# ArchieGertsman/spark-sched-sim

Measured on AMD Instinct MI355X. Metric: env-steps/sec at 4096 batched envs (TPC-H, 10 exec), higher is better.
Workload: dtype int64+f64

## Files before the change

### spark_sched_sim_amd/csrc/sss_sim.h

```cpp
#pragma once
#ifdef SSS_WIDE
#ifdef SSS_TIMELINE
#define SSS_KNAME(name) name##_wide_tl
#else
#define SSS_KNAME(name) name##_wide
#endif
#else
#ifdef SSS_TIMELINE
#define SSS_KNAME(name) name##_tl
#else
#define SSS_KNAME(name) name
#endif
#endif
#include "../../include/sss.h"
#include "sss_layout.h"
#include <wave_rt.h>


struct alignas(16) SssScratch {
  uint8_t pool8[8];
  uint8_t pool8b[8];
  uint64_t rng_buf[64];
  int32_t rng_pos, pad0_[3];
  uint8_t setA[SSS_SET_TABLE];
// ... 120 lines not shown
    if (H.err == 0) H.err = (code), H.err_line = (uint64_t)SSS_SRC_ID * 100000u + __LINE__; \
  } while (0)
#endif
#ifdef SSS_CHECK_TRACE
#define CHECK(cond)                                                                     \
  do {                                                                                  \
    if (!(cond)) {                                                                      \
      if (H.err == 0) fprintf(stderr, "[CHECK] line %d: %s\n", __LINE__, #cond);         \
      FAIL(SSS_ERR_INVARIANT);                                                          \
    }                                                                                   \
  } while (0)
#else
#define CHECK(cond)                          \
  do {                                       \
    if (!(cond)) FAIL(SSS_ERR_INVARIANT);     \
  } while (0)
#endif

#if defined(__HIP_DEVICE_COMPILE__) || defined(__clang__)
#define SSS_UNROLL4 _Pragma("unroll 4")
#define SSS_UNROLL8 _Pragma("unroll 8")
#else
#define SSS_UNROLL4
#define SSS_UNROLL8
#endif

#ifdef SSS_BATCH_STATS
extern "C" { extern long long sss_batch_stats[128]; }
#define STAT(i, v) ((void)(wave_lane() == 0 ? (sss_batch_stats[i] += (v)) : 0))
#else
#define STAT(i, v) ((void)0)
#endif

#include "sss_prof.h"
#if defined(SSS_CHECK_TRACE) && defined(SSS_UTRACE)
#define UTRACE(tag) do { if (wave_lane() < 2 && getenv("SSS_UTRACE")) fprintf(stderr, "[u] lane %d %s\n", wave_lane(), tag); } while (0)
#else
#define UTRACE(tag) ((void)0)
#endif

#define LENW_LEN 0x3FFFFFFF
#define SLOT_NONE 255
SSS_DEV uint16_t* lds_active() { return (uint16_t*)(g_pool + g_c.P.off_active); }
SSS_DEV uint8_t* lds_slot_of() { return g_pool + g_c.P.off_slot_of; }
SSS_DEV uint16_t* lds_keys() { return (uint16_t*)(g_pool + g_c.P.off_keys); }
SSS_DEV uint16_t* lds_jobset() { return (uint16_t*)(g_pool + g_c.P.off_jobset); }
SSS_DEV SssJob* lds_cjobs() { return (SssJob*)(g_pool + g_c.P.off_cjobs); }
SSS_DEV SssStage* lds_cstages() { return (SssStage*)(g_pool + g_c.P.off_cstages); }
SSS_DEV float* lds_cdur() { return (float*)(g_pool + g_c.P.off_cdur); }
SSS_DEV SssExDesc* lds_exdesc() { return (SssExDesc*)(g_pool + g_c.P.off_exdesc); }
SSS_DEV uint16_t* lds_old_active() { return (uint16_t*)(g_pool + g_c.P.off_old_active); }
SSS_DEV uint16_t* lds_slot_job() { return (uint16_t*)(g_pool + g_c.P.off_slot_job); }
SSS_DEV uint8_t* lds_slot_ref() { return g_pool + g_c.P.off_slot_ref; }

SSS_DEV SssJob* jobp(int j) {
  int s = lds_slot_of()[j];
  return s != SLOT_NONE ? lds_cjobs() + s : g_c.jobs + j;
}
SSS_DEV SssStage* stgp(int j, int st) {
  int s = lds_slot_of()[j];
  return s != SLOT_NONE ? lds_cstages() + s * g_c.SP + st : g_c.stages + j * g_c.SP + st;
}
SSS_DEV float* durp(int j, int st) {
  int s = lds_slot_of()[j];
  return s != SLOT_NONE ? lds_cdur() + s * g_c.SP + st : g_c.durations + j * g_c.SP + st;
}
// ... 443 lines not shown
```

### spark_sched_sim_amd/csrc/sss_sim_env.h

```cpp
#undef SSS_SRC_ID
#define SSS_SRC_ID 11
SSS_DEV void env_begin(const uint8_t* base) {
  PROF3(23);
  int lane = wave_lane();
  {
    const SssHot* g = (const SssHot*)base;
    if (lane < (int)(sizeof(SssHdr) / 16)) ((uint4*)&g_hot.h)[lane] = ((const uint4*)&g->h)[lane];
    for (int x = lane; x < SSS_MAX_EXEC; x += 64) {
      SssEvSlot ev;
      ev.t = __builtin_inf(), ev.seq = 0, ev.info = EV_NONE;
      uint32_t loc = POOL_NONE, csrc = 0, cdst = 0, cseq = 0;
      int16_t job = -1, cn = 0;
      int8_t ts = -1;
      uint8_t exe = 0;
      if (x < g_c.E)
        ev = g->ev[x], loc = g->ex_loc[x], job = g->ex_job[x], ts = g->ex_task_stage[x], exe = g->ex_executing[x], csrc = g->c_src[x],
        cdst = g->c_dst[x], cseq = g->c_seq[x], cn = g->c_n[x];
      g_hot.ev[x] = ev, g_hot.ex_loc[x] = loc, g_hot.ex_job[x] = job, g_hot.ex_task_stage[x] = ts, g_hot.ex_executing[x] = exe;
      g_hot.c_src[x] = csrc, g_hot.c_dst[x] = cdst, g_hot.c_seq[x] = cseq, g_hot.c_n[x] = cn;
    }
  }
  for (int i = lane; i < g_c.J_cap; i += 64) lds_slot_of()[i] = SLOT_NONE;
  for (int x = lane; x < g_c.E; x += 64) lds_exdesc()[x].gs = -1;
  lds_slot_ref()[lane] = 0;
// ... 27 lines not shown
      }
    }
    int nK = 0;
    for (int h = 0; h < SSS_EPL; h++) {
      key[h] = first[h] ? ((cnt[h] << 8) | (uint32_t)(64 * SSS_EPL - 1 - (lane + 64 * h))) : 0u;
      nK += popc64(wave_ballot(first[h]));
    }
    for (int h2 = 0; h2 < SSS_EPL; h2++)
      for (uint64_t fm = wave_ballot(first[h2]); fm; fm &= fm - 1) {
        const uint32_t kq = wave_readlane_u32(key[h2], ctz64_nz(fm));
        for (int h = 0; h < SSS_EPL; h++) rank[h] += kq > key[h] ? 1u : 0u;
      }
    const int n_used = nK < g_c.P.n_slots ? nK : g_c.P.n_slots;
    for (int h = 0; h < SSS_EPL; h++)
      if (first[h] && (int)rank[h] < g_c.P.n_slots) {
        lds_slot_of()[j[h]] = (uint8_t)rank[h];
        lds_slot_job()[rank[h]] = (uint16_t)j[h];
        lds_slot_ref()[rank[h]] = (uint8_t)cnt[h];
      }
    wave_sync();
    for (int h = 0; h < SSS_EPL; h++)
      if (has[h]) g_hot.ev[lane + 64 * h].info = info_with_slot(info[h], (uint32_t)lds_slot_of()[j[h]]);
    if (lane == 0) {
      uint64_t all = g_c.P.n_slots >= 64 ? ~0ull : (bit64(g_c.P.n_slots) - 1);
      uint64_t used = n_used >= 64 ? ~0ull : (bit64(n_used) - 1);
      g_sc.free_slots = all & ~used;
      g_sc.pending_free = -1, g_sc.pinned_job = -1, g_sc.idle_valid = 0, g_sc.fi_detach = 0;
      g_sc.events_this_step = 0;
      g_sc.active_version = 0, g_sc.old_version = 0, g_sc.jobset_valid = 0, g_sc.active_dirty = 0;
      g_sc.rng_pos = 64;
    }
  }
  wave_sync();
  uint64_t occ = ~g_sc.free_slots & (g_c.P.n_slots >= 64 ? ~0ull : (bit64(g_c.P.n_slots) - 1));
  int nK = popc64(occ);
  int per = 8 + g_c.SP + g_c.SP / 2;
  for (int i0 = lane; i0 < nK * per; i0 += 64 * 8) {
    uint64_t v[8];
    SSS_UNROLL8 for (int u = 0; u < 8; u++) {
      const int i = i0 + 64 * u;
      v[u] = 0;
      if (i < nK * per) {
        const int k = i / per, w = i - k * per;
        const int j = lds_slot_job()[k];
        v[u] = w < 8 ? ((const uint64_t*)(g_c.jobs + j))[w]
             : (w < 8 + g_c.SP ? ((const uint64_t*)(g_c.stages + j * g_c.SP))[w - 8] : ((const uint64_t*)(g_c.durations + j * g_c.SP))[w - 8 - g_c.SP]);
      }
    }
    SSS_UNROLL8 for (int u = 0; u < 8; u++) {
      const int i = i0 + 64 * u;
      if (i < nK * per) {
        const int k = i / per, w = i - k * per;
        if (w < 8)
          ((uint64_t*)(lds_cjobs() + k))[w] = v[u];
        else if (w < 8 + g_c.SP)
          ((uint64_t*)(lds_cstages() + k * g_c.SP))[w - 8] = v[u];
        else
          ((uint64_t*)(lds_cdur() + k * g_c.SP))[w - 8 - g_c.SP] = v[u];
      }
    }
  }
  wave_sync();
}

SSS_DEV void env_begin_readonly(const uint8_t* base) {
  int lane = wave_lane();
  const SssHot* g = (const SssHot*)base;
  if (lane < (int)(sizeof(SssHdr) / 16)) ((uint4*)&g_hot.h)[lane] = ((const uint4*)&g->h)[lane];
  for (int i = lane; i < g_c.J_cap; i += 64) lds_slot_of()[i] = SLOT_NONE;
  wave_sync();
  int A = g_hot.h.n_active;
  for (int i = lane; i < A; i += 64) lds_active()[i] = g_c.active_g[i];
  wave_sync();
}

SSS_DEV void env_end(uint8_t* base) {
  PROF3(24);
  int lane = wave_lane();
  wave_sync();
  if (lane == 0) rng_canonicalize();
  int A = g_hot.h.n_active;
  int per = 8 + g_c.SP + g_c.SP / 2;
  uint64_t occ = ~g_sc.free_slots & (g_c.P.n_slots >= 64 ? ~0ull : (bit64(g_c.P.n_slots) - 1));
  for (int i = lane; i < g_c.P.n_slots * per; i += 64) {
    int k = i / per, w = i - k * per;
    if (!(occ & bit64(k))) continue;
    int j = lds_slot_job()[k];
    if (w < 8)
      ((uint64_t*)(g_c.jobs + j))[w] = ((const uint64_t*)(lds_cjobs() + k))[w];
    else if (w < 8 + g_c.SP)
      ((uint64_t*)(g_c.stages + j * g_c.SP))[w - 8] = ((const uint64_t*)(lds_cstages() + k * g_c.SP))[w - 8];
    else
      ((uint64_t*)(g_c.durations + j * g_c.SP))[w - 8 - g_c.SP] = ((const uint64_t*)(lds_cdur() + k * g_c.SP))[w - 8 - g_c.SP];
  }
  if (g_sc.active_dirty)
// ... 15 lines not shown
  }
}


SSS_DEV void select_stage_wave(int stage_idx) {
  PROF3(34);
  const int lane = wave_lane();
  const int A = g_hot.h.n_active;
  int run = 0, fj = -1, fs = -1;
  for (int a0 = 0; a0 < A && stage_idx >= 0; a0 += 64) {
    const int a = a0 + lane;
    uint64_t m = 0;
    int jj = -1;
    if (a < A) jj = lds_active()[a], m = jobp(jj)->sched_mask;
    const uint32_t n = (uint32_t)popc64(m);
    const int lo = run + (int)wave_scan_excl_u32(n);
    run += (int)wave_sum_u32(n);
    const bool mine = stage_idx >= lo && stage_idx < lo + (int)n;
    const uint64_t hit = wave_ballot(mine);
    if (hit) {
      if (mine) {
        for (int i = 0; i < stage_idx - lo; i++) m &= m - 1;
        g_sc.sel_job = jj, g_sc.sel_stage = ctz64(m);
      }
      fj = 0;
      break;
    }
  }
  if (fj < 0 && lane == 0) g_sc.sel_job = -1, g_sc.sel_stage = -1;
  (void)fs;
  wave_sync();
}

SSS_DEV bool take_action(int stage_idx, int num_exec) {
  PROF3(17);
  if (stage_idx < -1 || stage_idx >= H.obs_n_nodes || num_exec < 1 || num_exec > g_c.E) {
    H.err = SSS_ERR_ACTION_SPACE;
    return false;
  }
  if (stage_idx == -1) {
    commit_remaining_executors();
    return true;
  }
  if (stage_idx >= H.obs_n_sched) {
    H.err = SSS_ERR_STAGE_IDX;
    return false;
  }
  if (num_exec > trk_num_committable()) {
    H.err = SSS_ERR_TOO_MANY;
    return false;
  }
  const int j = g_sc.sel_job, s = g_sc.sel_stage;
  CHECK(j >= 0);
  if (j < 0) return false;
  SssStage st = (*stgp(j, s));
  int demand = (int)st.remaining - ((int)st.moving_to + (int)st.commit_to);
  int n = num_exec < demand ? num_exec : demand;
  CHECK(n > 0);
  trk_add_commitment(n, key_stage_pool(j, s));
  SssJob& job = (*jobp(j));
  job.selected_mask |= bit64(s);
  int old_n = popc64(job.sched_mask);
  uint64_t m = 0;
  if (job_passes_filter(j, trk_source_job_id())) m = ready_mask_of_job(job, false);
  job.sched_mask = m;
  H.n_sched += popc64(m) - old_n;
  return true;
}

SSS_DEV void jobtime_build_set() {
  PROF3(18);
  SetImg<uint16_t> all;
  all.tab = lds_jobset();
  for (int i = 0; i < 8; i++) all.tab[i] = 0;
  all.mask = 7, all.fill = 0, all.used = 0, all.finger = 0, all.cap = 0xFFFFFFFFu, all.big = nullptr, all.small = nullptr, all.wide = false;
  for (int k = 0; k < g_sc.n_old_active; k++) set_add(all, (uint32_t)lds_old_active()[k], lds_keys());
  for (int k = 0; k < H.n_active; k++) set_add(all, (uint32_t)lds_active()[k], lds_keys());
  g_sc.jobset_mask = (int32_t)all.mask;
}

SSS_DEV void jobtime_build_set_wave() {
  const int lane = wave_lane();
  uint16_t* tab = lds_jobset();
  const int cap = g_c.P.jobset_slots;
  const int n_old = g_sc.n_old_active, n_act = g_hot.h.n_active;
  for (int i = lane * 8; i < cap; i += 64 * 8) *(uint4*)(tab + i) = mk_u4(0u, 0u, 0u, 0u);
  wave_sync();
  uint32_t not_max = 0xFFFFFFFFu;
  for (int k = lane; k < n_old + n_act; k += 64) {
    const uint32_t id = k < n_old ? lds_old_active()[k] : lds_active()[k - n_old];
    tab[id] = (uint16_t)(id + 2);
    not_max = ~id < not_max ? ~id : not_max;
  }
  wave_sync();
  uint32_t cnt = 0;
  for (int i = lane * 8; i < cap; i += 64 * 8) {
    const uint4 q = *(const uint4*)(tab + i);
    const uint32_t w[4] = {q.x, q.y, q.z, q.w};
    for (int b = 0; b < 4; b++) cnt += ((w[b] & 0xFFFFu) != 0 ? 1u : 0u) + ((w[b] >> 16) != 0 ? 1u : 0u);
// ... 136 lines not shown
          handled = fast_run<FUSED>(f);
        } else if (tasks_left) {
          handled = fast_run<FUSED>(f);
        } else {
#ifndef SSS_NO_BATCH
          if (64 - g_sc.rng_pos < rng_need) {
            rng_refill();
          }
#endif
          handled = tf ? batch_released_events(f, ex) : batch_arrival_events(f, ex);
#ifndef SSS_NO_LEAN
          if (handled == 0) handled = tf ? lean_released(f, ex, t_win, info_win) : lean_arrival(f, ex, t_win, info_win);
#endif
          if (handled == 0 && tf) preflush_completing_job(f, info_win, t_win);
        }
        if (handled > 0) continue;
      }
      if (lane == 0) status = handle_popped(f, ex, t_win, info_win, t_slow);
      status = (int)wave_lane0_u32((uint32_t)status);
    } while (status == 0);
    if (lane == 0) {
      g_sc.f_done = status == 1, g_sc.f_scan = status == 2;
      H.prof[0] += t_slow;
    }
    wave_sync();
    if (g_sc.f_done) {
      if (lane == 0) {
        for (int a = 0; a < H.n_active; a++) (*jobp(lds_active()[a])).sched_mask = 0;
        H.n_sched = 0;
      }
      wave_sync();
      return false;
    }
    int n = find_schedulable_all();
    if (n > 0) {
      if (lane == 0) H.n_sched = n;
      wave_sync();
      return false;
    }
    publish_idle_mask();
    if (lane == 0) {
      move_idle_executors_all(POOL_NONE);
      H.curr_source = POOL_NONE;
      g_sc.idle_valid = 0;
    }
    wave_sync();
  }
}

SSS_DEV void do_reset(const SssLayout& L, uint64_t seed, double time_limit) {
  PROF3(27);
  int lane = wave_lane();
  SssHot& hot = g_hot;
  for (int i = lane; i < g_c.J_cap; i += 64) lds_slot_of()[i] = SLOT_NONE;
  lds_slot_ref()[lane] = 0;
  wave_sync();
  if (lane == 0) {
    g_sc.free_slots = g_c.P.n_slots >= 64 ? ~0ull : (bit64(g_c.P.n_slots) - 1);
    g_sc.pending_free = -1, g_sc.pinned_job = -1, g_sc.idle_valid = 0, g_sc.fi_detach = 0;
    uint64_t n_steps = H.n_steps, n_events = H.n_events, model_bytes = H.model_bytes;
    int dur_head = H.dur_head, dur_n = H.dur_n, episodes = H.episodes, last_ep_steps = H.last_ep_steps;
    double last_ep_return = H.last_ep_return, last_ep_wall = H.last_ep_wall;
    uint64_t prof[5];
    for (int i = 0; i < 5; i++) prof[i] = H.prof[i];
    uint64_t n_fast_keep = H.n_fast, n_batched_keep = H.n_batched, n_rounds_keep = H.n_rounds, pad0_keep = H.err_line;
    SssHdr z = {};
    H = z;
// ... 121 lines not shown
    g_sc.wall_old = H.wall_old, g_sc.n_old_active = H.n_old_active;
    g_sc.old_version = g_sc.active_version, g_sc.jobset_valid = 0;
    H.mid_step = 0;
  }
  wave_sync();
}
SSS_DEV void step_yield() {
  const int lane = wave_lane();
  for (int a = lane; a < g_sc.n_old_active; a += 64) g_c.active_g[g_c.J_cap + a] = lds_old_active()[a];
  if (lane == 0) H.mid_step = 1, H.step_events = g_sc.events_this_step, H.wall_old = g_sc.wall_old, H.n_old_active = g_sc.n_old_active;
  wave_sync();
}

template <bool FUSED = false>
SSS_DEV double do_step(int stage_idx, int num_exec, int budget = 0, bool* yielded = nullptr) {
  PROF3(28);
  int lane = wave_lane();
  uint64_t t0 = wave_clock();
  const bool go_on = wave_ballot(g_hot.h.mid_step != 0) != 0;
  uint64_t t1 = t0;
  if (go_on) {
    step_continue();
  } else {
  publish_idle_mask();
  select_stage_wave(stage_idx);
  if (lane == 0) {
    g_sc.f_round_continues = 1, g_sc.f_fulfil = 0;
    g_sc.events_this_step = 0, g_sc.events_at_launch = 0;
    H.last_reward = 0.0;
    if (H.need_reset || H.terminated) {
      H.err = SSS_ERR_NEED_RESET;
    } else {
      H.err = 0;
      bool ok = take_action(stage_idx, num_exec);
      if (ok && !H.err) {
        H.n_steps++;
        H.ep_steps++;
        if (!(trk_num_committable() > 0 && H.n_sched > 0)) {
          commit_remaining_executors();
          g_sc.f_fulfil = 1;
        }
      }
    }
    if (!g_sc.f_fulfil) g_sc.idle_valid = 0;
  }
  wave_sync();
  if (g_sc.f_fulfil) {
    fulfil_order_commitments();
    if (lane == 0) {
      fulfil_build_list();
      g_sc.idle_valid = 0;
    }
    wave_sync();
    fulfil_run();
    if (lane == 0) {
      H.curr_source = POOL_NONE;
      g_sc.wall_old = H.wall_time;
      g_sc.n_old_active = H.n_active;
      g_sc.old_version = g_sc.active_version;
      g_sc.f_round_continues = 0;
    }
  }
  if (lane == 0 && H.err && H.err != SSS_ERR_ACTION_SPACE && H.err != SSS_ERR_STAGE_IDX && H.err != SSS_ERR_TOO_MANY) H.need_reset = 1;
  wave_sync();
  t1 = wave_clock();
  if (lane == 0) H.prof[1] += t1 - t0;
  if (wave_ballot(g_sc.f_round_continues || g_hot.h.err) != 0) return 0.0;
  for (int a = lane; a < g_hot.h.n_active; a += 64) {
    int j = lds_active()[a];
    (*jobp(j)).selected_mask = 0;
    lds_old_active()[a] = (uint16_t)j;
  }
  wave_sync();
  }
  if (resume_simulation<FUSED>(budget)) {
    step_yield();
    *yielded = true;
    return 0.0;
  }
  return step_reward(t1, wave_clock());
}

SSS_DEV double step_reward(uint64_t t1, uint64_t t2) {
  const int lane = wave_lane();
  if (lane == 0) {
    g_sc.f_need_jobtime = 0;
    if (!H.err && H.wall_time - g_sc.wall_old != 0.0) {
// ... 31 lines not shown
```

### spark_sched_sim_amd/csrc/sss_sim_events.h

```cpp
#undef SSS_SRC_ID
#define SSS_SRC_ID 6

SSS_DEV void cache_release(int j) {
  int k = lds_slot_of()[j];
  if (k == SLOT_NONE) return;
  g_c.jobs[j] = lds_cjobs()[k];
  for (int s = 0; s < g_c.SP; s++) {
    g_c.stages[j * g_c.SP + s] = lds_cstages()[k * g_c.SP + s];
    g_c.durations[j * g_c.SP + s] = lds_cdur()[k * g_c.SP + s];
  }
  lds_slot_of()[j] = SLOT_NONE;
  g_sc.free_slots |= bit64(k);
}
SSS_DEV int cache_acquire(int j) {
  PROF3(19);
  int k = lds_slot_of()[j];
  if (k != SLOT_NONE) return k;
  if (g_sc.free_slots == 0) {
    int victim = -1;
    for (int q = 0; q < g_c.P.n_slots; q++)
      if (lds_slot_ref()[q] == 0 && (int)lds_slot_job()[q] != g_sc.pinned_job) {
        victim = q;
        break;
      }
    if (victim < 0) return SLOT_NONE;
    cache_release((int)lds_slot_job()[victim]);
  }
  k = ctz64(g_sc.free_slots);
  g_sc.free_slots &= g_sc.free_slots - 1;
  lds_cjobs()[k] = g_c.jobs[j];
  {
    const uint64_t* gs = (const uint64_t*)(g_c.stages + j * g_c.SP);
    const uint64_t* gd = (const uint64_t*)(g_c.durations + j * g_c.SP);
    uint64_t* ls = (uint64_t*)(lds_cstages() + k * g_c.SP);
    uint64_t* ld = (uint64_t*)(lds_cdur() + k * g_c.SP);
    const int nw = g_c.SP + g_c.SP / 2;
    for (int w0 = 0; w0 < nw; w0 += 8) {
      uint64_t v[8];
      SSS_UNROLL8 for (int u = 0; u < 8; u++) {
        const int w = w0 + u;
        v[u] = w < g_c.SP ? gs[w < g_c.SP ? w : 0] : (w < nw ? gd[w - g_c.SP] : 0ull);
      }
      SSS_UNROLL8 for (int u = 0; u < 8; u++) {
        const int w = w0 + u;
        if (w < g_c.SP) ls[w] = v[u];
        else if (w < nw) ld[w - g_c.SP] = v[u];
      }
    }
  }
  lds_slot_of()[j] = (uint8_t)k;
  lds_slot_job()[k] = (uint16_t)j;
  lds_slot_ref()[k] = 0;
  return k;
}

SSS_DEV void handle_job_arrival(int j) {
  lds_active()[H.n_active] = (uint16_t)j;
  H.n_active++;
  g_sc.active_version++, g_sc.active_dirty = 1;
  H.graph_version++;
  if (g_c.pool_hdr[0].used > 0) H.curr_source = POOL_COMMON;
}

SSS_DEV void handle_executor_arrival(int e, int j, int s) {
  PROF3(14);
  const JobView v = jobview(j);
  CHECK(g_hot.ex_task_stage[e] < 0);
  v.job->local_mask = local_with(v.job->local_mask, e);
  g_hot.ex_job[e] = (int16_t)j;
  tl_append(e, H.wall_time, j);
  const int mv = (int)v.st[s].moving_to - 1;
  CHECK(mv >= 0);
  v.st[s].moving_to = (uint8_t)mv;
  update_sat(v, s);
  trk_move_executor_to_pool(e, key_job_pool(j), false);
  move_executor_to_stage(e, j, s);
}

SSS_DEV void process_job_completion(int j) {
  PROF3(15);
  if (pool_size(key_job_pool(j)) > 0) move_idle_executors_all(key_job_pool(j));
  CHECK(pool_size(key_job_pool(j)) == 0);
  int k;
  for (k = 0; k < H.n_active; k++)
    if (lds_active()[k] == j) break;
  CHECK(k < H.n_active);
// ... 186 lines not shown
```

### spark_sched_sim_amd/csrc/sss_sim_fulfil.h

```cpp
#undef SSS_SRC_ID
#define SSS_SRC_ID 5
SSS_DEV int fulfil_chunk(int c0, int n, int& serial_end) {
  PROF3(35);
  const int lane = wave_lane();
  const bool active = lane < n;
  const int idx = c0 + (active ? lane : 0);
  const uint32_t src = g_hot.h.curr_source;
  const uint32_t counter0 = g_hot.h.counter, h0 = g_hot.h.rng_has32, u32_0 = g_hot.h.rng_u32;
  const int pos = g_sc.rng_pos;
  const double wall = g_hot.h.wall_time;
  const int e = g_sc.fi_e[idx], k = g_sc.fi_k[idx];
  const uint32_t dst = g_sc.fc_dst[k];
  const int j = key_job(dst), s = key_stage(dst);
  const int exj = g_hot.ex_job[e], exts = g_hot.ex_task_stage[e];
  const int src_job = key_job(src);
  SssStage* sp = stgp(j, s);
  SssJob* jp = jobp(j);
  SssStage st = *sp;
  const uint64_t local = jp->local_mask;
  const int gs = jp->gs_base + s;
  const bool in_frontier = (jp->frontier_mask & bit64(s)) != 0;
  const int slot = lds_slot_of()[j];
  const SssPoolHdr src_hdr = g_c.pool_hdr[pool_index(src)];
  const int type = exj != j ? FI_SEND : (in_frontier ? FI_EXEC : FI_PARK);
// ... 253 lines not shown
    pool_pair_flush_one(src, so);
    pool_pair_flush_one(dstp, sn);
  }
  if (lane == 0) {
    SssHdr& h = g_hot.h;
    if (!moves) {
      SssPoolHdr* hd = g_c.pool_hdr + pool_index(src);
      hd->commit_from = (int16_t)(hd->commit_from - n);
      CHECK(hd->commit_from >= 0);
    }
    if (j >= 0) {
      h.supply_none -= n;
      CHECK(h.supply_none >= 0);
    }
    g_hot.c_n[ci] = (int16_t)c_left;
    if (c_left == 0) {
      const int last = h.n_commits - 1;
      g_hot.c_src[ci] = g_hot.c_src[last], g_hot.c_dst[ci] = g_hot.c_dst[last], g_hot.c_n[ci] = g_hot.c_n[last], g_hot.c_seq[ci] = g_hot.c_seq[last];
      h.n_commits = last;
    }
    if (moves) {
      for (int i = from; i < to; i++) {
        const int e = g_sc.fi_e[i];
        g_hot.ex_loc[e] = dstp;
        if (dstp == POOL_COMMON) g_hot.ex_job[e] = -1, g_hot.ex_task_stage[e] = -1, tl_append(e, h.wall_time, -1);
      }
      if (dstp == POOL_COMMON) local_group_detach(jp, moved);
    }
  }
  wave_sync();
  return true;
}

SSS_DEV void fulfil_run() {
  PROF3(33);
  const int m = g_sc.fi_m, m_par = g_sc.fi_m_par;
  int done = 0;
#ifndef SSS_NO_BATCH
  while (done < m_par) {
    if (64 - g_sc.rng_pos < 48) rng_refill();
    int n = m_par - done < 24 ? m_par - done : 24;
    if (wave_lane() == 0)
      for (int i = done; i < done + n; i++) cache_acquire(key_job(g_sc.fc_dst[g_sc.fi_k[i]]));
    wave_sync();
    int serial_end = 0;
    int got = fulfil_chunk(done, n, serial_end);
    if (got < n) {
      STAT(54, 1);
      if (got > 0) {
        int dummy = 0;
        int again = fulfil_chunk(done, got, dummy);
        if (again < got) break;
        STAT(53, 1), STAT(55, got);
        done += got;
      }
      if (wave_lane() == 0) fulfil_serial_range(done, serial_end);
      wave_sync();
      if (wave_ballot(g_hot.h.err != 0) != 0) break;
      done = serial_end;
      continue;
    }
    STAT(53, 1), STAT(55, n);
    done += n;
  }
  if (done == m_par && m_par < m && wave_ballot(g_hot.h.err != 0) == 0 && fulfil_common_wave(m_par, m)) {
    STAT(123, 1), STAT(124, m - m_par);
    done = m;
  }
#endif
  STAT(56, m - done);
  (void)m_par;
  if (wave_lane() == 0 && done < m) fulfil_serial(done);
  wave_sync();
}

SSS_DEV void commit_remaining_executors() {
  int n = trk_num_committable();
// ... 3 lines not shown
```

### spark_sched_sim_amd/csrc/sss_sim_jobs.h

```cpp
#undef SSS_SRC_ID
#define SSS_SRC_ID 4

SSS_DEV void job_attach_executor(int j, int e) {
  CHECK(g_hot.ex_task_stage[e] < 0);
  SssJob* jp = jobp(j);
  jp->local_mask = local_with(jp->local_mask, e);
  g_hot.ex_job[e] = (int16_t)j;
}
SSS_DEV void job_detach_executor(int j, int e) {
  SssJob* jp = jobp(j);
  CHECK(local_has(jp->local_mask, e));
  jp->local_mask = local_without(jp->local_mask, e);
  g_hot.ex_job[e] = -1;
  g_hot.ex_task_stage[e] = -1;
}
SSS_DEV bool stage_completed(const SssStage& st) { return st.remaining == 0 && st.executing == 0; }

SSS_DEV bool job_record_stage_completion(int j, int s) {
  PROF3(4);
  SssJob& job = (*jobp(j));
  CHECK((job.active_mask & bit64(s)) && (job.frontier_mask & bit64(s)));
  uint64_t active = job.active_mask & ~bit64(s);
  job.active_mask = active;
  uint64_t frontier = job.frontier_mask & ~bit64(s);
// ... 31 lines not shown
#endif
  return eff + (((size_t)gs * 8 + li) * 3 + mode) * 4;
}

SSS_DEV double task_duration(const SssJob* job, int s, int e) {
  PROF3(5);
  int gs = job->gs_base + s;
  int n_local = local_count(job->local_mask);
  CHECK(n_local > 0 && n_local <= g_c.E);
  if (n_local <= 0 || n_local > g_c.E) return 0.0;
  int li, ri;
  executor_interval(n_local, li, ri);
  if (li != ri) {
    double left = (double)exec_level_value(li), right = (double)exec_level_value(ri);
    int rand_pt = 1 + (int)(rng_random() * (right - left));
    if (!((double)rand_pt <= (double)n_local - left)) li = ri;
  }
  int task_stage = g_hot.ex_task_stage[e];
  int mode = task_stage < 0 ? 0 : (task_stage == s ? 1 : 2);
  const int32_t* d = eff_row(g_c.pk.eff, gs, li, mode);
  int off = d[0], lenw = d[1];
  int len = lenw & 0x3FFFFFFF;
  if (len == 0) {
    FAIL(SSS_ERR_NO_DURATION);
    return 0.0;
  }
  uint32_t i = rng_integers((uint32_t)len);
  double v = (double)g_c.pk.durations[off + (int)i];
  if (lenw >> 30) v += g_c.P.warmup_delay;
  return v;
}


SSS_DEV uint64_t ready_mask_of_job(const SssJob& job, bool first_only) {
  uint64_t cand = job.active_mask & ~job.selected_mask & ~job.sat_mask;
  uint64_t m = 0;
  while (cand) {
    int s = ctz64(cand);
    cand &= cand - 1;
    uint64_t parents = g_c.pk.stage_parent_mask[job.gs_base + s];
    if ((parents & ~job.sat_mask) == 0) {
      m |= bit64(s);
      if (first_only) break;
    }
  }
  return m;
}

SSS_DEV bool job_passes_filter(int j, int source_job_id) {
  return j == source_job_id || (int)(*jobp(j)).supply < g_c.E;
}

SSS_DEV void find_backup_stage(int e, int& out_j, int& out_s) {
  PROF3(6);
  out_j = -1, out_s = -1;
  int ejob = g_hot.ex_job[e];
  CHECK(ejob >= 0);
  if (ejob < 0) return;
  int src = ejob <= 0 ? trk_source_job_id() : ejob;
  if (job_passes_filter(ejob, src)) {
    uint64_t m = ready_mask_of_job((*jobp(ejob)), true);
    if (m) {
      out_j = ejob, out_s = ctz64(m);
      return;
    }
  }
  bool ejob_active = (*jobp(ejob)).active_mask != 0;
  int n_others = H.n_active - (ejob_active ? 1 : 0);
  for (int a = 0; a < H.n_active; a++) {
    int j = lds_active()[a];
    if (n_others > 0 && j == ejob) continue;
    if (!job_passes_filter(j, src)) continue;
    uint64_t m = ready_mask_of_job((*jobp(j)), true);
    if (m) {
      out_j = j, out_s = ctz64(m);
      return;
    }
  }
}


#define INFO_SLOT_NONE 127u
SSS_DEV uint32_t ev_info(int kind, int j, int s, uint32_t slot) {
  return (uint32_t)kind | ((uint32_t)s << 8) | ((slot > 63u ? INFO_SLOT_NONE : slot) << 14) | ((uint32_t)j << 21);
}
SSS_DEV int info_kind(uint32_t i) { return (int)(i & 0xFF); }
SSS_DEV int info_stage(uint32_t i) { return (int)((i >> 8) & 0x3F); }
SSS_DEV uint32_t info_slot(uint32_t i) { return (i >> 14) & 0x7F; }
SSS_DEV int info_job(uint32_t i) { return (int)(i >> 21); }
SSS_DEV uint32_t info_with_slot(uint32_t i, uint32_t slot) { return (i & ~(0x7Fu << 14)) | ((slot > 63u ? INFO_SLOT_NONE : slot) << 14); }

SSS_DEV int cache_acquire(int j);
SSS_DEV void push_event(int e, double t, int kind, int j, int s) {
  SssHot& hot = g_hot;
  CHECK((hot.ev[e].info & 0xFF) == EV_NONE);
  int slot = cache_acquire(j);
  if (slot != SLOT_NONE) lds_slot_ref()[slot]++;
  SssEvSlot sl;
  sl.t = t, sl.seq = H.counter++, sl.info = ev_info(kind, j, s, (uint32_t)slot);
  hot.ev[e] = sl;
}

SSS_DEV void execute_next_task(int e, int j, int s) {
  PROF3(7);
  const JobView v = jobview(j);
  SssStage st = v.st[s];
  CHECK(st.remaining > 0 && g_hot.ex_job[e] == j && !g_hot.ex_executing[e]);
  st.remaining = (st.remaining - 1);
  st.executing = (int16_t)(st.executing + 1);
  v.st[s] = st;
  if (st.remaining == 0) v.job->sat_count = (int16_t)(v.job->sat_count + 1);
  {
    const int demand = (int)st.remaining - ((int)st.moving_to + (int)st.commit_to);
    const uint64_t m = v.job->sat_mask;
    v.job->sat_mask = demand <= 0 ? (m | bit64(s)) : (m & ~bit64(s));
  }
  double d = task_duration(v.job, s, e);
  g_hot.ex_task_stage[e] = (int8_t)s;
  g_hot.ex_executing[e] = 1;
  v.dur[s] = (float)d;
  push_event(e, H.wall_time + d, EV_TASK_FINISHED, j, s);
}

SSS_DEV void send_executor(int e, int j, int s) {
  PROF3(8);
// ... 221 lines not shown
```

### spark_sched_sim_amd/csrc/sss_sim_observe.h

```cpp
#undef SSS_SRC_ID
#define SSS_SRC_ID 10
SSS_DEV int find_schedulable_all() {
  PROF3(21);
  int lane = wave_lane();
  int A = g_sc.m_n_active;
  int src_job = g_sc.m_src_job;
  uint32_t total = 0;
  for (int a0 = 0; a0 < A; a0 += 64) {
    int a = a0 + lane;
    uint32_t cnt = 0;
    if (a < A) {
      int j = lds_active()[a];
      SssJob* job = jobp(j);
      uint64_t m = 0;
      if (j == src_job || (int)job->supply < g_c.E) m = ready_mask_of_job(*job, false);
      job->sched_mask = m;
      cnt = (uint32_t)popc64(m);
    }
    total += wave_sum_u32(cnt);
  }
  return (int)total;
}

SSS_DEV void write_observation(const SssLayout& L, const SssBuffers& B, int env, double reward) {
  PROF3(22);
  int lane = wave_lane();
  uint64_t t_obs0 = wave_clock();
  const SssHdr& h = g_hot.h;
  float* __restrict__ nodes = B.nodes + (size_t)env * L.n_cap * 3;
  int32_t* __restrict__ el = B.edge_links + (size_t)env * L.ed_cap * 2;
  int32_t* __restrict__ dag_ptr = B.dag_ptr + (size_t)env * (L.J_cap + 1);
  int32_t* __restrict__ sup = B.exec_supplies + (size_t)env * L.J_cap;
  int A = h.n_active;
  uint32_t srck = h.curr_source;
  int src_job = (srck == POOL_NONE || srck == POOL_COMMON) ? -1 : key_job(srck);
  int src_idx = A;
  uint64_t lt = bit64(lane) - 1;
  uint16_t* nbase = lds_keys();
  uint32_t run = 0;
  for (int a0 = 0; a0 < A; a0 += 64) {
    int a = a0 + lane;
    uint32_t cnt = 0;
    int j = -1, supply = 0;
    if (a < A) {
      j = lds_active()[a];
      const SssJob* job = jobp(j);
      cnt = (uint32_t)popc64(job->active_mask);
      supply = job->supply;
// ... 101 lines not shown
```

### spark_sched_sim_amd/csrc/sss_sim_tracker.h

```cpp
#undef SSS_SRC_ID
#define SSS_SRC_ID 3

SSS_DEV int trk_source_job_id() {
  uint32_t k = H.curr_source;
  if (k == POOL_NONE || k == POOL_COMMON) return -1;
  return key_job(k);
}

SSS_DEV void publish_scan_inputs() {
  g_sc.m_n_active = H.n_active;
  g_sc.m_src_job = trk_source_job_id();
}

SSS_DEV int trk_num_committable() {
  uint32_t k = H.curr_source;
  if (k == POOL_NONE) return 0;
  int p = pool_index(k);
  int n = (int)g_c.pool_hdr[p].used - (int)g_c.pool_hdr[p].commit_from;
  CHECK(n >= 0);
  return n;
}

SSS_DEV void update_sat(const JobView& v, int s) {
  const SssStage st = v.st[s];
  const int demand = (int)st.remaining - ((int)st.moving_to + (int)st.commit_to);
  const uint64_t m = v.job->sat_mask;
  v.job->sat_mask = demand <= 0 ? (m | bit64(s)) : (m & ~bit64(s));
}
SSS_DEV void update_sat(int j, int s) { update_sat(jobview(j), s); }

SSS_DEV void add_supply(int job, int d) {
  if (job < 0) {
    H.supply_none += d;
    CHECK(H.supply_none >= 0);
  } else {
    SssJob* jp = jobp(job);
    int v = (int)jp->supply + d;
    CHECK(v >= 0);
    jp->supply = (int16_t)v;
  }
}

SSS_DEV void trk_add_commitment(int n, uint32_t dst) {
  PROF3(1);
  uint32_t src = H.curr_source;
  CHECK(src != POOL_NONE);
  if (src == POOL_NONE) return;
  SssHot& hot = g_hot;
  int i;
  for (i = 0; i < H.n_commits; i++)
    if (hot.c_src[i] == src && hot.c_dst[i] == dst) break;
  if (i < H.n_commits)
    hot.c_n[i] = (int16_t)(hot.c_n[i] + n);
  else {
    CHECK(i < SSS_MAX_EXEC);
    if (i >= SSS_MAX_EXEC) return;
    hot.c_src[i] = src, hot.c_dst[i] = dst, hot.c_n[i] = (int16_t)n, hot.c_seq[i] = H.commit_seq++;
    H.n_commits = i + 1;
  }
  int ps = pool_index(src);
  g_c.pool_hdr[ps].commit_from = (int16_t)(g_c.pool_hdr[ps].commit_from + n);
  CHECK((int)g_c.pool_hdr[ps].used >= (int)g_c.pool_hdr[ps].commit_from);
  int dj = key_job(dst), ds = key_stage(dst);
  if (ds >= 0) {
    const JobView v = jobview(dj);
    v.st[ds].commit_to = (uint8_t)(v.st[ds].commit_to + n);
    update_sat(v, ds);
  }
  if (dj != key_job(src)) add_supply(dj, n);
}

SSS_DEV uint32_t trk_remove_commitment(int e, uint32_t dst) {
  PROF3(2);
  SssHot& hot = g_hot;
  uint32_t src = hot.ex_loc[e];
  CHECK(src != POOL_NONE);
  int i;
  for (i = 0; i < H.n_commits; i++)
    if (hot.c_src[i] == src && hot.c_dst[i] == dst) break;
  CHECK(i < H.n_commits);
  if (i >= H.n_commits) return src;
  hot.c_n[i] = (int16_t)(hot.c_n[i] - 1);
  int ps = pool_index(src);
  g_c.pool_hdr[ps].commit_from = (int16_t)(g_c.pool_hdr[ps].commit_from - 1);
  CHECK(g_c.pool_hdr[ps].commit_from >= 0);
  int dj = key_job(dst), ds = key_stage(dst);
  if (ds >= 0) {
    const JobView v = jobview(dj);
    const int c = (int)v.st[ds].commit_to - 1;
    CHECK(c >= 0);
    v.st[ds].commit_to = (uint8_t)c;
    update_sat(v, ds);
// ... 263 lines not shown
```

Measured before the change: 24.07 million.

## Batch cache fills in fulfil, inline take_action commit, chunk ready-mask parent loads

In the step path, lane 0 now only assigns cache slots; the newly assigned slots are then filled by all lanes in one wave-wide pass, instead of lane 0 acquiring and loading each job serially. take_action gains a specialised step path that inlines commitment bookkeeping on local copies of the job and stage, and returns the remaining committable count so it is not recomputed. ready_mask_of_job gains a chunked variant that gathers several parent masks before testing them, to overlap the loads. The cost is more template variants and duplicated logic, plus some risk of divergence between the fused and unfused paths.

After: 24.26 million (median of 6 runs). Within noise of the previous version (+0.8%).

```diff
diff --git a/spark_sched_sim_amd/csrc/sss_sim.h b/spark_sched_sim_amd/csrc/sss_sim.h
--- a/spark_sched_sim_amd/csrc/sss_sim.h
+++ b/spark_sched_sim_amd/csrc/sss_sim.h
@@ -176,6 +176,8 @@
 #define STAT(i, v) ((void)0)
 #endif
 
+#define SSS_READY_CHUNK 8
+
 #include "sss_prof.h"
 #if defined(SSS_CHECK_TRACE) && defined(SSS_UTRACE)
 #define UTRACE(tag) do { if (wave_lane() < 2 && getenv("SSS_UTRACE")) fprintf(stderr, "[u] lane %d %s\n", wave_lane(), tag); } while (0)
diff --git a/spark_sched_sim_amd/csrc/sss_sim_env.h b/spark_sched_sim_amd/csrc/sss_sim_env.h
--- a/spark_sched_sim_amd/csrc/sss_sim_env.h
+++ b/spark_sched_sim_amd/csrc/sss_sim_env.h
@@ -83,35 +83,7 @@
     }
   }
   wave_sync();
-  uint64_t occ = ~g_sc.free_slots & (g_c.P.n_slots >= 64 ? ~0ull : (bit64(g_c.P.n_slots) - 1));
-  int nK = popc64(occ);
-  int per = 8 + g_c.SP + g_c.SP / 2;
-  for (int i0 = lane; i0 < nK * per; i0 += 64 * 8) {
-    uint64_t v[8];
-    SSS_UNROLL8 for (int u = 0; u < 8; u++) {
-      const int i = i0 + 64 * u;
-      v[u] = 0;
-      if (i < nK * per) {
-        const int k = i / per, w = i - k * per;
-        const int j = lds_slot_job()[k];
-        v[u] = w < 8 ? ((const uint64_t*)(g_c.jobs + j))[w]
-             : (w < 8 + g_c.SP ? ((const uint64_t*)(g_c.stages + j * g_c.SP))[w - 8] : ((const uint64_t*)(g_c.durations + j * g_c.SP))[w - 8 - g_c.SP]);
-      }
-    }
-    SSS_UNROLL8 for (int u = 0; u < 8; u++) {
-      const int i = i0 + 64 * u;
-      if (i < nK * per) {
-        const int k = i / per, w = i - k * per;
-        if (w < 8)
-          ((uint64_t*)(lds_cjobs() + k))[w] = v[u];
-        else if (w < 8 + g_c.SP)
-          ((uint64_t*)(lds_cstages() + k * g_c.SP))[w - 8] = v[u];
-        else
-          ((uint64_t*)(lds_cdur() + k * g_c.SP))[w - 8 - g_c.SP] = v[u];
-      }
-    }
-  }
-  wave_sync();
+  cache_fill<true>(popc64(~g_sc.free_slots & (g_c.P.n_slots >= 64 ? ~0ull : (bit64(g_c.P.n_slots) - 1))));
 }
 
 SSS_DEV void env_begin_readonly(const uint8_t* base) {
@@ -193,25 +165,68 @@
   wave_sync();
 }
 
-SSS_DEV bool take_action(int stage_idx, int num_exec) {
+template <bool kStep>
+SSS_DEV bool take_action(int stage_idx, int num_exec, int& left) {
   PROF3(17);
+  left = 0;
   if (stage_idx < -1 || stage_idx >= H.obs_n_nodes || num_exec < 1 || num_exec > g_c.E) {
     H.err = SSS_ERR_ACTION_SPACE;
     return false;
   }
   if (stage_idx == -1) {
     commit_remaining_executors();
+    left = trk_num_committable();
     return true;
   }
   if (stage_idx >= H.obs_n_sched) {
     H.err = SSS_ERR_STAGE_IDX;
     return false;
   }
+  const int j = g_sc.sel_job, s = g_sc.sel_stage;
+  const uint32_t src = H.curr_source;
+  if (kStep && src != POOL_NONE && j >= 0) {
+    SssPoolHdr* const hd = g_c.pool_hdr + pool_index(src);
+    const JobView v = jobview(j);
+    const int used = (int)hd->used;
+    int commit_from = (int)hd->commit_from;
+    SssStage st = v.st[s];
+    SssJob job = *v.job;
+    CHECK(used - commit_from >= 0);
+    if (num_exec > used - commit_from) {
+      H.err = SSS_ERR_TOO_MANY;
+      return false;
+    }
+    const int demand = (int)st.remaining - ((int)st.moving_to + (int)st.commit_to);
+    const int n = num_exec < demand ? num_exec : demand;
+    CHECK(n > 0);
+    if (trk_commitment_entry(src, key_stage_pool(j, s), n)) {
+      commit_from = (int)(int16_t)(commit_from + n);
+      hd->commit_from = (int16_t)commit_from;
+      CHECK(used >= commit_from);
+      st.commit_to = (uint8_t)(st.commit_to + n);
+      v.st[s] = st;
+      const int demand_now = (int)st.remaining - ((int)st.moving_to + (int)st.commit_to);
+      job.sat_mask = demand_now <= 0 ? (job.sat_mask | bit64(s)) : (job.sat_mask & ~bit64(s));
+      if (j != key_job(src)) {
+        const int sup = (int)job.supply + n;
+        CHECK(sup >= 0);
+        job.supply = (int16_t)sup;
+      }
+    }
+    job.selected_mask |= bit64(s);
+    const int old_n = popc64(job.sched_mask);
+    uint64_t m = 0;
+    if (j == trk_source_job_id() || (int)job.supply < g_c.E) m = ready_mask_of_job<SSS_READY_CHUNK>(job, false);
+    job.sched_mask = m;
+    v.job->sat_mask = job.sat_mask, v.job->supply = job.supply, v.job->selected_mask = job.selected_mask, v.job->sched_mask = m;
+    H.n_sched += popc64(m) - old_n;
+    left = used - commit_from;
+    return true;
+  }
   if (num_exec > trk_num_committable()) {
     H.err = SSS_ERR_TOO_MANY;
     return false;
   }
-  const int j = g_sc.sel_job, s = g_sc.sel_stage;
   CHECK(j >= 0);
   if (j < 0) return false;
   SssStage st = (*stgp(j, s));
@@ -226,6 +241,7 @@
   if (job_passes_filter(j, trk_source_job_id())) m = ready_mask_of_job(job, false);
   job.sched_mask = m;
   H.n_sched += popc64(m) - old_n;
+  left = trk_num_committable();
   return true;
 }
 
@@ -428,7 +444,7 @@
       wave_sync();
       return false;
     }
-    int n = find_schedulable_all();
+    int n = find_schedulable_all<FUSED ? 1 : SSS_READY_CHUNK>();
     if (n > 0) {
       if (lane == 0) H.n_sched = n;
       wave_sync();
@@ -616,11 +632,12 @@
       H.err = SSS_ERR_NEED_RESET;
     } else {
       H.err = 0;
-      bool ok = take_action(stage_idx, num_exec);
+      int left = 0;
+      bool ok = take_action<!FUSED>(stage_idx, num_exec, left);
       if (ok && !H.err) {
         H.n_steps++;
         H.ep_steps++;
-        if (!(trk_num_committable() > 0 && H.n_sched > 0)) {
+        if (!(left > 0 && H.n_sched > 0)) {
           commit_remaining_executors();
           g_sc.f_fulfil = 1;
         }
@@ -636,7 +653,7 @@
       g_sc.idle_valid = 0;
     }
     wave_sync();
-    fulfil_run();
+    fulfil_run<!FUSED>();
     if (lane == 0) {
       H.curr_source = POOL_NONE;
       g_sc.wall_old = H.wall_time;
diff --git a/spark_sched_sim_amd/csrc/sss_sim_events.h b/spark_sched_sim_amd/csrc/sss_sim_events.h
--- a/spark_sched_sim_amd/csrc/sss_sim_events.h
+++ b/spark_sched_sim_amd/csrc/sss_sim_events.h
@@ -52,6 +52,72 @@
   lds_slot_job()[k] = (uint16_t)j;
   lds_slot_ref()[k] = 0;
   return k;
+}
+
+SSS_DEV int cache_assign(int j, uint64_t& fresh) {
+  PROF3(19);
+  int k = lds_slot_of()[j];
+  if (k != SLOT_NONE) return k;
+  if (g_sc.free_slots == 0) {
+    int victim = -1;
+    for (int q = 0; q < g_c.P.n_slots; q++)
+      if (lds_slot_ref()[q] == 0 && (int)lds_slot_job()[q] != g_sc.pinned_job) {
+        victim = q;
+        break;
+      }
+    if (victim < 0) return SLOT_NONE;
+    if (fresh & bit64(victim)) {
+      lds_slot_of()[lds_slot_job()[victim]] = SLOT_NONE;
+      g_sc.free_slots |= bit64(victim);
+      fresh &= ~bit64(victim);
+    } else {
+      cache_release((int)lds_slot_job()[victim]);
+    }
+  }
+  k = ctz64(g_sc.free_slots);
+  g_sc.free_slots &= g_sc.free_slots - 1;
+  lds_slot_of()[j] = (uint8_t)k;
+  lds_slot_job()[k] = (uint16_t)j;
+  lds_slot_ref()[k] = 0;
+  fresh |= bit64(k);
+  return k;
+}
+
+template <bool kDense>
+SSS_DEV void cache_fill(int n_fill) {
+  wave_sync();
+  const int lane = wave_lane();
+  const int per = 8 + g_c.SP + g_c.SP / 2;
+  const int n_words = n_fill * per;
+  for (int i0 = lane; i0 < n_words; i0 += 64 * 8) {
+    uint64_t v[8];
+    int slot[8];
+    SSS_UNROLL8 for (int u = 0; u < 8; u++) {
+      const int i = i0 + 64 * u;
+      v[u] = 0, slot[u] = 0;
+      if (i < n_words) {
+        const int q = i / per, w = i - q * per;
+        const int k = kDense ? q : (int)g_sc.rl_idx[q];
+        slot[u] = k;
+        const int j = lds_slot_job()[k];
+        v[u] = w < 8 ? ((const uint64_t*)(g_c.jobs + j))[w]
+             : (w < 8 + g_c.SP ? ((const uint64_t*)(g_c.stages + j * g_c.SP))[w - 8] : ((const uint64_t*)(g_c.durations + j * g_c.SP))[w - 8 - g_c.SP]);
+      }
+    }
+    SSS_UNROLL8 for (int u = 0; u < 8; u++) {
+      const int i = i0 + 64 * u;
+      if (i < n_words) {
+        const int k = kDense ? i / per : slot[u], w = i - (i / per) * per;
+        if (w < 8)
+          ((uint64_t*)(lds_cjobs() + k))[w] = v[u];
+        else if (w < 8 + g_c.SP)
+          ((uint64_t*)(lds_cstages() + k * g_c.SP))[w - 8] = v[u];
+        else
+          ((uint64_t*)(lds_cdur() + k * g_c.SP))[w - 8 - g_c.SP] = v[u];
+      }
+    }
+  }
+  wave_sync();
 }
 
 SSS_DEV void handle_job_arrival(int j) {
diff --git a/spark_sched_sim_amd/csrc/sss_sim_fulfil.h b/spark_sched_sim_amd/csrc/sss_sim_fulfil.h
--- a/spark_sched_sim_amd/csrc/sss_sim_fulfil.h
+++ b/spark_sched_sim_amd/csrc/sss_sim_fulfil.h
@@ -309,6 +309,7 @@
   return true;
 }
 
+template <bool kStep = false>
 SSS_DEV void fulfil_run() {
   PROF3(33);
   const int m = g_sc.fi_m, m_par = g_sc.fi_m_par;
@@ -317,9 +318,19 @@
   while (done < m_par) {
     if (64 - g_sc.rng_pos < 48) rng_refill();
     int n = m_par - done < 24 ? m_par - done : 24;
-    if (wave_lane() == 0)
-      for (int i = done; i < done + n; i++) cache_acquire(key_job(g_sc.fc_dst[g_sc.fi_k[i]]));
-    wave_sync();
+    if (kStep) {
+      uint32_t n_fresh = 0;
+      if (wave_lane() == 0) {
+        uint64_t fresh = 0;
+        for (int i = done; i < done + n; i++) cache_assign(key_job(g_sc.fc_dst[g_sc.fi_k[i]]), fresh);
+        for (; fresh; fresh &= fresh - 1) g_sc.rl_idx[n_fresh++] = (uint8_t)ctz64(fresh);
+      }
+      cache_fill<false>((int)wave_lane0_u32(n_fresh));
+    } else {
+      if (wave_lane() == 0)
+        for (int i = done; i < done + n; i++) cache_acquire(key_job(g_sc.fc_dst[g_sc.fi_k[i]]));
+      wave_sync();
+    }
     int serial_end = 0;
     int got = fulfil_chunk(done, n, serial_end);
     if (got < n) {
diff --git a/spark_sched_sim_amd/csrc/sss_sim_jobs.h b/spark_sched_sim_amd/csrc/sss_sim_jobs.h
--- a/spark_sched_sim_amd/csrc/sss_sim_jobs.h
+++ b/spark_sched_sim_amd/csrc/sss_sim_jobs.h
@@ -87,7 +87,29 @@
 }
 
 
+template <int kChunk = 1>
 SSS_DEV uint64_t ready_mask_of_job(const SssJob& job, bool first_only) {
+  if (kChunk > 1) {
+    const uint64_t sat = job.sat_mask;
+    uint64_t cand = job.active_mask & ~job.selected_mask & ~sat;
+    const uint64_t* parent_mask = g_c.pk.stage_parent_mask + job.gs_base;
+    uint64_t m = 0;
+    while (cand) {
+      int s[kChunk];
+      uint64_t parents[kChunk];
+      int last = ctz64(cand);
+      SSS_UNROLL8 for (int u = 0; u < kChunk; u++) {
+        s[u] = cand ? ctz64(cand) : last;
+        last = s[u];
+        cand &= cand - 1;
+      }
+      SSS_UNROLL8 for (int u = 0; u < kChunk; u++) parents[u] = parent_mask[s[u]];
+      SSS_UNROLL8 for (int u = 0; u < kChunk; u++)
+        if ((parents[u] & ~sat) == 0) m |= bit64(s[u]);
+      if (first_only && m) break;
+    }
+    return first_only ? (m & (0 - m)) : m;
+  }
   uint64_t cand = job.active_mask & ~job.selected_mask & ~job.sat_mask;
   uint64_t m = 0;
   while (cand) {
@@ -146,6 +168,9 @@
 SSS_DEV uint32_t info_with_slot(uint32_t i, uint32_t slot) { return (i & ~(0x7Fu << 14)) | ((slot > 63u ? INFO_SLOT_NONE : slot) << 14); }
 
 SSS_DEV int cache_acquire(int j);
+SSS_DEV int cache_assign(int j, uint64_t& fresh);
+template <bool kDense>
+SSS_DEV void cache_fill(int n_fill);
 SSS_DEV void push_event(int e, double t, int kind, int j, int s) {
   SssHot& hot = g_hot;
   CHECK((hot.ev[e].info & 0xFF) == EV_NONE);
diff --git a/spark_sched_sim_amd/csrc/sss_sim_observe.h b/spark_sched_sim_amd/csrc/sss_sim_observe.h
--- a/spark_sched_sim_amd/csrc/sss_sim_observe.h
+++ b/spark_sched_sim_amd/csrc/sss_sim_observe.h
@@ -1,5 +1,6 @@
 #undef SSS_SRC_ID
 #define SSS_SRC_ID 10
+template <int kChunk = 1>
 SSS_DEV int find_schedulable_all() {
   PROF3(21);
   int lane = wave_lane();
@@ -13,7 +14,7 @@
       int j = lds_active()[a];
       SssJob* job = jobp(j);
       uint64_t m = 0;
-      if (j == src_job || (int)job->supply < g_c.E) m = ready_mask_of_job(*job, false);
+      if (j == src_job || (int)job->supply < g_c.E) m = ready_mask_of_job<kChunk>(*job, false);
       job->sched_mask = m;
       cnt = (uint32_t)popc64(m);
     }
diff --git a/spark_sched_sim_amd/csrc/sss_sim_tracker.h b/spark_sched_sim_amd/csrc/sss_sim_tracker.h
--- a/spark_sched_sim_amd/csrc/sss_sim_tracker.h
+++ b/spark_sched_sim_amd/csrc/sss_sim_tracker.h
@@ -41,11 +41,7 @@
   }
 }
 
-SSS_DEV void trk_add_commitment(int n, uint32_t dst) {
-  PROF3(1);
-  uint32_t src = H.curr_source;
-  CHECK(src != POOL_NONE);
-  if (src == POOL_NONE) return;
+SSS_DEV bool trk_commitment_entry(uint32_t src, uint32_t dst, int n) {
   SssHot& hot = g_hot;
   int i;
   for (i = 0; i < H.n_commits; i++)
@@ -54,10 +50,19 @@
     hot.c_n[i] = (int16_t)(hot.c_n[i] + n);
   else {
     CHECK(i < SSS_MAX_EXEC);
-    if (i >= SSS_MAX_EXEC) return;
+    if (i >= SSS_MAX_EXEC) return false;
     hot.c_src[i] = src, hot.c_dst[i] = dst, hot.c_n[i] = (int16_t)n, hot.c_seq[i] = H.commit_seq++;
     H.n_commits = i + 1;
   }
+  return true;
+}
+
+SSS_DEV void trk_add_commitment(int n, uint32_t dst) {
+  PROF3(1);
+  uint32_t src = H.curr_source;
+  CHECK(src != POOL_NONE);
+  if (src == POOL_NONE) return;
+  if (!trk_commitment_entry(src, dst, n)) return;
   int ps = pool_index(src);
   g_c.pool_hdr[ps].commit_from = (int16_t)(g_c.pool_hdr[ps].commit_from + n);
   CHECK((int)g_c.pool_hdr[ps].used >= (int)g_c.pool_hdr[ps].commit_from);
```
